# linusmossberg/monte-carlo-ray-tracer

Measured on NVIDIA H100. Metric: Mray/s (primary+shadow+bounce), higher is better.
Workload: dtype f64

## Files before the change

monte-carlo-ray-tracer_b200/csrc/abi.cu:

```cuda
#include <algorithm>
#include <cmath>
#include <cstdio>
#include <cstdlib>
#include <cstring>
#include <string>
#include <vector>

#include "mcrt_abi.h"
#include "launch.h"
#include "bvh_build.h"
#include "image.h"
#include "denoise.h"

using namespace mcrt;

static const int MCRT_INTERNAL_EMIT = 100;

#define CK(call)                                                                              \
    do {                                                                                      \
        cudaError_t e_ = (call);                                                              \
        if (e_ != cudaSuccess)                                                                \
        {                                                                                     \
            ctx->error = std::string(#call) + ": " + cudaGetErrorString(e_);                  \
            return MCRT_ERR_CUDA;                                                             \
// ... 489 lines not shown
        for (uint32_t i = 0; i < s.n_prims; i++)
        {
            if (s.prim_type[i] == MCRT_PRIM_SPHERE && d.prims_class == PRIMS_TRI) d.prims_class = PRIMS_TRI_SPHERE;
            else if (s.prim_type[i] != MCRT_PRIM_TRIANGLE && s.prim_type[i] != MCRT_PRIM_SPHERE) { d.prims_class = PRIMS_ALL; break; }
        }
        d.material_flags_any = 0;
        for (const auto& m : a.materials) d.material_flags_any |= m.flags;
        d.scene_ior = (R)s.scene_ior;
        d.scene_scale = (R)ctx->scene_scale;
        return MCRT_OK;
    }

    template <class R>
    int ensureWave(mcrt_ctx* ctx, WaveBuffers<R>& w, std::vector<void*>& track)
    {
        if (w.capacity == ctx->pool_paths) return MCRT_OK;
        freeAll(track);
        w.capacity = 0;
        const size_t n = ctx->pool_paths;
        int rc;
        for (int b = 0; b < 2; b++)
        {
            if ((rc = devAlloc(ctx, track, &w.buf[b].ray_o, n))) return rc;
            if ((rc = devAlloc(ctx, track, &w.buf[b].ray_d, n))) return rc;
            if ((rc = devAlloc(ctx, track, &w.buf[b].thr, n))) return rc;
            if ((rc = devAlloc(ctx, track, &w.buf[b].iors_a, n))) return rc;
            if ((rc = devAlloc(ctx, track, &w.buf[b].iors_b, n))) return rc;
            if ((rc = devAlloc(ctx, track, &w.buf[b].meta, n))) return rc;
            if ((rc = devAlloc(ctx, track, &w.buf[b].meta2, n))) return rc;
        }
        if ((rc = devAlloc(ctx, track, &w.shadow, n))) return rc;
        if ((rc = devAlloc(ctx, track, &w.hits, n))) return rc;
        w.capacity = ctx->pool_paths;
        return MCRT_OK;
    }

    int ensureSort(mcrt_ctx* ctx)
    {
        if (ctx->sort_capacity == ctx->pool_paths) return MCRT_OK;
        freeAll(ctx->sort_allocs);
        ctx->sort_capacity = 0;
        const size_t n = ctx->pool_paths;
        int rc;
        RaySort& r = ctx->sort;
        for (int b = 0; b < 2; b++)
        {
            if ((rc = devAlloc(ctx, ctx->sort_allocs, &r.path_key[b], n))) return rc;
            if ((rc = devAlloc(ctx, ctx->sort_allocs, &r.path_rank[b], n))) return rc;
        }
        if ((rc = devAlloc(ctx, ctx->sort_allocs, &r.path_order, n))) return rc;
        if ((rc = devAlloc(ctx, ctx->sort_allocs, &r.shadow_key, n))) return rc;
        if ((rc = devAlloc(ctx, ctx->sort_allocs, &r.shadow_rank, n))) return rc;
        if ((rc = devAlloc(ctx, ctx->sort_allocs, &r.shadow_order, n))) return rc;
        if ((rc = devAlloc(ctx, ctx->sort_allocs, &r.shade_key, n))) return rc;
        if ((rc = devAlloc(ctx, ctx->sort_allocs, &r.shade_rank, n))) return rc;
        if ((rc = devAlloc(ctx, ctx->sort_allocs, &r.shade_order, n))) return rc;
        if ((rc = devAlloc(ctx, ctx->sort_allocs, &r.hist_shade, (size_t)SORT_BINS))) return rc;
        if ((rc = devAlloc(ctx, ctx->sort_allocs, &r.hist_path, (size_t)SORT_BINS))) return rc;
        if ((rc = devAlloc(ctx, ctx->sort_allocs, &r.hist_shadow, (size_t)SORT_BINS))) return rc;
        if ((rc = devAlloc(ctx, ctx->sort_allocs, &r.bin_start, (size_t)SORT_BINS))) return rc;
        if ((rc = devAlloc(ctx, ctx->sort_allocs, &r.block_offset, (size_t)2 * SORT_SCAN_BLOCKS))) return rc;
        if ((rc = devAlloc(ctx, ctx->sort_allocs, &r.done_counter, (size_t)1))) return rc;
        CK(cudaMemset(r.done_counter, 0, sizeof(uint32_t)));
        ctx->sort_capacity = ctx->pool_paths;
        return MCRT_OK;
    }

    int ensureFilm(mcrt_ctx* ctx, size_t values)
    {
        if (ctx->film_values >= values && ctx->d_film) return MCRT_OK;
        if (ctx->d_film) cudaFree(ctx->d_film);
        ctx->d_film = nullptr; ctx->film_values = 0;
        CK(cudaMalloc((void**)&ctx->d_film, values * sizeof(double)));
        ctx->film_values = values;
        return MCRT_OK;
    }

    template <class R> DeviceScene<R>& sceneOf(mcrt_ctx* ctx);
    template <> DeviceScene<double>& sceneOf<double>(mcrt_ctx* ctx) { return ctx->scene64; }
    template <> DeviceScene<float>& sceneOf<float>(mcrt_ctx* ctx) { return ctx->scene32; }
    template <class R> WaveBuffers<R>& waveOf(mcrt_ctx* ctx);
    template <> WaveBuffers<double>& waveOf<double>(mcrt_ctx* ctx) { return ctx->wave64; }
    template <> WaveBuffers<float>& waveOf<float>(mcrt_ctx* ctx) { return ctx->wave32; }
    template <class R> std::vector<void*>& waveAllocsOf(mcrt_ctx* ctx);
    template <> std::vector<void*>& waveAllocsOf<double>(mcrt_ctx* ctx) { return ctx->wave_allocs64; }
    template <> std::vector<void*>& waveAllocsOf<float>(mcrt_ctx* ctx) { return ctx->wave_allocs32; }

    void fillStats(mcrt_stats* st, const Counters& c, uint64_t iterations, uint64_t launches, double ms)
    {
        if (!st) return;
        std::memset(st, 0, sizeof(*st));
        st->paths = c.paths;
        st->extension_rays = c.extension_rays;
        st->shadow_rays = c.shadow_rays;
        st->box_tests = c.box_tests;
        st->prim_tests = c.prim_tests;
        st->knn_queries = c.knn_queries;
        st->wavefront_iterations = iterations;
        st->kernel_launches = launches;
        st->ior_stack_overflows = c.ior_stack_overflows;
        st->max_depth = c.max_depth;
        st->gpu_ms_total = ms;
        st->shadow_box_tests = c.shadow_box_tests;
        st->shadow_prim_tests = c.shadow_prim_tests;
        st->extend_work_sum = c.work_sum;
        st->extend_work_warpmax = c.work_warpmax;
        st->replayed_rays = c.replayed_rays;
    }
// ... 162 lines not shown
        CK(cudaEventRecord(ctx->ev_start, s));
        CK(cudaMemcpyAsync(ctx->d_counters, &ctx->h_counters[0], sizeof(Counters), cudaMemcpyHostToDevice, s));
        if (!accum)
        {
            CK(cudaMemsetAsync(ctx->d_film, 0, film_pixels * 3 * sizeof(double), s));
            if (filtered) CK(cudaMemsetAsync(ctx->d_film_wsum, 0, film_pixels * sizeof(double), s));
        }
        const bool sorting = ctx->sort_rays != 0;
        if (sorting)
        {
            CK(cudaMemsetAsync(p.sort.hist_path, 0, SORT_BINS * sizeof(uint32_t), s));
            CK(cudaMemsetAsync(p.sort.hist_shadow, 0, SORT_BINS * sizeof(uint32_t), s));
            CK(cudaMemsetAsync(ctx->sort.hist_shade, 0, SORT_BINS * sizeof(uint32_t), s));
        }
        auto sortPaths = [&](int buffer)
        {
            launchSortScan(p.sort.hist_path, p.sort, s);
            launchSortScatter(p.sort.path_key[buffer], p.sort.path_rank[buffer], p.sort, p.sort.path_order,
                              &ctx->d_counters->n_cur, grid, s);
        };

        uint64_t launches = 0, iterations = 0;

        if (emitting) Launch<R>::emitGenerate(p, 0, grid, s);
        else Launch<R>::generate(p, 0, grid, s);
        launchAdvance(ctx->d_counters, s);
        launches += 2;
        if (sorting) { sortPaths(0); launches += 2; }

        int pending[2] = { 0, 0 };
        int slot = 0;
        bool done = false;
        while (!done)
        {
            for (int k = 0; k < ctx->poll_interval; k++)
            {
                const int cur = (int)(iterations & 1u);
                cudaEvent_t* ev = nullptr;
                if (ctx->stage_timing)
                {
                    while (ctx->stage_events.size() < 6 * (iterations + 1))
                    {
                        cudaEvent_t e;
                        CK(cudaEventCreate(&e));
                        ctx->stage_events.push_back(e);
                    }
                    ev = &ctx->stage_events[6 * iterations];
                    cudaEventRecord(ev[0], s);
                }
                Launch<R>::extend(p, cur, grid, s);
                if (ev) cudaEventRecord(ev[1], s);
                if (p.sort.shade_order)
                {
                    Launch<R>::shadeKey(p, grid, s);
                    launchSortScan(p.sort.hist_shade, p.sort, s);
                    launchSortScatter(p.sort.shade_key, p.sort.shade_rank, p.sort, p.sort.shade_order, &ctx->d_counters->n_cur, grid, s);
                    launches += 3;
                }
                if (emitting)
                {
                    Launch<R>::emitShade(p, cur, grid, s);
                }
                else if (integrator == MCRT_INTEGRATOR_PHOTON)
                {
                    Launch<R>::shadePhoton(p, cur, grid, s);
                    if (ev) cudaEventRecord(ev[5], s);
                    Launch<R>::knn(p, grid, s);
                    launches += 1;
                }
                else
                {
                    Launch<R>::shade(p, cur, grid, s);
                }
                if (ev) cudaEventRecord(ev[2], s);
                if (!emitting)
                {
                    if (sorting)
                    {
                        launchSortScan(p.sort.hist_shadow, p.sort, s);
                        launchSortScatter(p.sort.shadow_key, p.sort.shadow_rank, p.sort, p.sort.shadow_order,
                                          &ctx->d_counters->n_shadow, grid, s);
                        launches += 2;
                    }
                    Launch<R>::shadow(p, grid, s);
                }
                if (ev) cudaEventRecord(ev[3], s);
                if (emitting) Launch<R>::emitGenerate(p, cur ^ 1, grid, s);
                else Launch<R>::generate(p, cur ^ 1, grid, s);
                launchAdvance(ctx->d_counters, s);
                if (sorting) { sortPaths(cur ^ 1); launches += 2; }
                if (ev) cudaEventRecord(ev[4], s);
                launches += 5;
                iterations++;
            }
            CK(cudaMemcpyAsync(&ctx->h_counters[slot], ctx->d_counters, sizeof(Counters), cudaMemcpyDeviceToHost, s));
            CK(cudaEventRecord(ctx->ev_poll[slot], s));
            pending[slot] = 1;
            const int other = slot ^ 1;
            if (pending[other])
            {
                CK(cudaEventSynchronize(ctx->ev_poll[other]));
                const Counters& c = ctx->h_counters[other];
                if (c.n_cur == 0 && c.next_work >= c.total_work) done = true;
                pending[other] = 0;
            }
            slot = other;
        }

        if (!emitting && !accum)
        {
// ... 1514 lines not shown
```

monte-carlo-ray-tracer_b200/csrc/integrator.cuh:

```cuda
#pragma once

#include "bsdf.cuh"
#include "intersect.cuh"
#include "bvh4.cuh"
#include "photon.cuh"
#include "film.cuh"
#include "mcrt_abi.h"

#ifndef MCRT_TRACE_MINBLOCKS_F64
#define MCRT_TRACE_MINBLOCKS_F64 2
#endif
#ifndef MCRT_TRACE_MINBLOCKS_F32
#define MCRT_TRACE_MINBLOCKS_F32 4
#endif
#ifndef MCRT_TRACE_MINBLOCKS_F64_PRUNED
#define MCRT_TRACE_MINBLOCKS_F64_PRUNED 4
#endif
#ifndef MCRT_TRACE_MINBLOCKS_FAST
#define MCRT_TRACE_MINBLOCKS_FAST 2
#endif
#ifndef MCRT_TRACE_MINBLOCKS_DYN
#define MCRT_TRACE_MINBLOCKS_DYN 4
#endif
#ifndef MCRT_KNN_MINBLOCKS
#define MCRT_KNN_MINBLOCKS 8
#endif
#ifndef MCRT_GATHER_MINBLOCKS
#define MCRT_GATHER_MINBLOCKS 3
#endif
#ifndef MCRT_SHADE_MINBLOCKS
#define MCRT_SHADE_MINBLOCKS 3
#endif
#ifndef MCRT_SHADE_MINBLOCKS_LITE
#define MCRT_SHADE_MINBLOCKS_LITE 3
#endif
#ifndef MCRT_SORT_ORIGIN_BITS
#define MCRT_SORT_ORIGIN_BITS 4
#endif
#ifndef MCRT_SORT_DIR_Q
#define MCRT_SORT_DIR_Q 1
#endif

namespace mcrt
{
    constexpr int IOR_STACK_CAPACITY = 8;

    struct Counters
    {
        uint32_t n_cur, n_next, n_shadow, n_gen;
        unsigned long long next_work, total_work;
        unsigned long long paths, extension_rays, shadow_rays, box_tests, prim_tests, knn_queries;
        unsigned long long shadow_box_tests, shadow_prim_tests;
        unsigned long long ior_stack_overflows;
        unsigned long long replayed_rays;
        uint32_t fetch_extend, fetch_shadow;
        uint32_t traversal_overflow, max_depth;
        uint32_t n_knn, _pad;
        unsigned long long work_sum, work_warpmax;
        unsigned long long n_photons[2];
        uint32_t photon_overflow, _pad2;
    };

    template <class R> struct PathBuffer
    {
        V4<R>* ray_o;
        V4<R>* ray_d;
        V4<R>* thr;
        V4<R>* iors_a;
        V4<R>* iors_b;
        uint4* meta;
        uint4* meta2;
    };

    template <class R> struct alignas(16 * sizeof(R)) ShadowRecord
    {
        V4<R> o;
        V4<R> d;
        uint4 meta;
        V4<R> k;
    };
    static_assert(sizeof(ShadowRecord<double>) == 128 && sizeof(ShadowRecord<float>) == 64, "one shadow record per line");
    static_assert(offsetof(ShadowRecord<double>, k) == 96, "the float64 padding is the 16-byte chunk 5 (k_shade writes it)");

    constexpr uint32_t SORT_ORIGIN_BITS = MCRT_SORT_ORIGIN_BITS;
    constexpr uint32_t SORT_DIR_Q = MCRT_SORT_DIR_Q;
    constexpr uint32_t SORT_DIR_BITS = 3 + 2 * SORT_DIR_Q;
    constexpr uint32_t SORT_KEY_BITS = 3 * SORT_ORIGIN_BITS + SORT_DIR_BITS;
    constexpr uint32_t SORT_BINS = 1u << SORT_KEY_BITS;

    struct RaySort
    {
        uint32_t* path_key[2];
        uint32_t* path_rank[2];
        uint32_t* path_order;
        uint32_t* shadow_key;
        uint32_t* shadow_rank;
        uint32_t* shadow_order;
        uint32_t* hist_path;
        uint32_t* hist_shadow;
        uint32_t* bin_start;
        uint32_t* block_offset;
        uint32_t* done_counter;
        uint32_t shade_sorted;
        uint32_t* shade_key;
        uint32_t* shade_rank;
        uint32_t* shade_order;
        uint32_t* hist_shade;
        uint32_t prim_scale;
        float key_min[3], key_scale[3];
    };

    MCRT_D uint32_t spreadBits3(uint32_t v)
    {
        v = (v | (v << 16)) & 0x030000FFu;
        v = (v | (v << 8)) & 0x0300F00Fu;
        v = (v | (v << 4)) & 0x030C30C3u;
        v = (v | (v << 2)) & 0x09249249u;
        return v;
    }

    template <class R>
    MCRT_D uint32_t rayKey(const RaySort& rs, const V3<R>& o, const V3<R>& d, uint32_t src_prim)
    {
        uint32_t cell;
        if (rs.prim_scale && src_prim != NO_PRIM)
        {
            cell = (uint32_t)(((unsigned long long)src_prim * rs.prim_scale) >> 32);
        }
        else
        {
            constexpr float CELLS = (float)(1u << SORT_ORIGIN_BITS);
            float cx = ((float)o.x - rs.key_min[0]) * rs.key_scale[0];
            float cy = ((float)o.y - rs.key_min[1]) * rs.key_scale[1];
            float cz = ((float)o.z - rs.key_min[2]) * rs.key_scale[2];
            uint32_t ix = (uint32_t)fminf(fmaxf(cx, 0.0f), CELLS - 1.0f);
            uint32_t iy = (uint32_t)fminf(fmaxf(cy, 0.0f), CELLS - 1.0f);
            uint32_t iz = (uint32_t)fminf(fmaxf(cz, 0.0f), CELLS - 1.0f);
            cell = spreadBits3(ix) | (spreadBits3(iy) << 1) | (spreadBits3(iz) << 2);
        }
        float dx = (float)d.x, dy = (float)d.y, dz = (float)d.z;
        float ax = fabsf(dx), ay = fabsf(dy), az = fabsf(dz);
        uint32_t face; float u, v, m;
        if (ax >= ay && ax >= az) { face = dx < 0.0f ? 1u : 0u; u = dy; v = dz; m = ax; }
        else if (ay >= az)        { face = dy < 0.0f ? 3u : 2u; u = dx; v = dz; m = ay; }
        else                      { face = dz < 0.0f ? 5u : 4u; u = dx; v = dy; m = az; }
        constexpr float Q = (float)(1u << SORT_DIR_Q);
        float inv = m > 0.0f ? 0.5f * Q / m : 0.0f;
        uint32_t qu = (uint32_t)fminf(fmaxf(u * inv + 0.5f * Q, 0.0f), Q - 1.0f);
        uint32_t qv = (uint32_t)fminf(fmaxf(v * inv + 0.5f * Q, 0.0f), Q - 1.0f);
        uint32_t dir = (face << (2 * SORT_DIR_Q)) | (qu << SORT_DIR_Q) | qv;
        return (dir << (3 * SORT_ORIGIN_BITS)) | cell;
    }

    MCRT_D uint32_t sortRank(uint32_t* hist, uint32_t key, bool pred)
    {
        const unsigned active = __ballot_sync(0xFFFFFFFFu, pred);
        uint32_t rank = 0;
        if (pred)
// ... 255 lines not shown
            {
            const unsigned long long w = base_work + j;
            uint32_t pixel, sample, film_index;
            V3<R> start, direction;
            if (p.user_rays)
            {
                pixel = p.user_pixel[w];
                sample = p.user_sample[w];
                film_index = (uint32_t)w;
                const double* r = p.user_rays + 6 * w;
                start = V3<R>((R)r[0], (R)r[1], (R)r[2]);
                direction = V3<R>((R)r[3], (R)r[4], (R)r[5]);
            }
            else
            {
                uint32_t local = (uint32_t)(w % p.n_pixels);
                if constexpr (LIST) local = p.pixel_list[local];
                sample = (uint32_t)(w / p.n_pixels);
                const uint32_t row = local / p.camera.width, col = local - row * p.camera.width;
                pixel = (p.row_first + row * p.row_step) * p.camera.width + col;
                film_index = local;
                SamplerState smp = SamplerState::make(p.global_seed, pixel, sample, 0u);
                cameraRay(p.camera, p.scene.scene_ior, pixel, smp, start, direction);
                if constexpr (FILM) filmSplatSampleWeight(p.filmp, p.global_seed, pixel, sample);
            }
            stStream(&out.ray_o[slot], V4<R>(start, p.scene.scene_ior));
            stStream(&out.ray_d[slot], V4<R>(direction, R(1)));
            stStream(&out.thr[slot], V4<R>(R(1), R(1), R(1), R(0)));
            stStream(&out.meta[slot], make_uint4(pixel, sample, 0u, 0u));
            stStream(&out.meta2[slot], make_uint4(NO_PRIM, 1u, film_index, NO_PRIM));
            if (p.sort.path_order) key = rayKey(p.sort, start, direction, NO_PRIM);
            }
            if (p.sort.path_order)
            {
                const uint32_t rank = sortRank(p.sort.hist_path, key, valid);
                if (valid) { p.sort.path_key[next][slot] = key; p.sort.path_rank[next][slot] = rank; }
            }
        }
    }

    static __global__ void k_advance(Counters* c)
    {
        c->n_cur = c->n_next + c->n_gen;
        c->next_work += c->n_gen;
        c->paths += c->n_gen;
        c->n_next = 0;
        c->n_gen = 0;
        c->n_shadow = 0;
        c->n_knn = 0;
        c->fetch_extend = 0;
        c->fetch_shadow = 0;
    }

    template <class R, int PRIMS, int FAST>
    __global__ void __launch_bounds__(256, FAST == 2 ? MCRT_TRACE_MINBLOCKS_DYN : (FAST == 1 ? MCRT_TRACE_MINBLOCKS_FAST : (PRIMS == PRIMS_ALL ? Mode<R>::trace_minblocks : Mode<R>::trace_minblocks_pruned))) k_extend(WaveParams<R> p, int cur)
    {
        const uint32_t n = p.counters->n_cur;
        const PathBuffer<R>& in = p.buf[cur];
        TraceCounters cnt = { 0u, 0u, 0u };
        uint32_t overflow = 0;
        unsigned long long rays = 0;
        const uint32_t* order = p.sort.path_order;
        if constexpr (Mode<R>::parity && FAST == 2)
        {
            traceManyFast<PRIMS>(p.scene, n, &p.counters->fetch_extend,
                [&](uint32_t ii, RayQ<R>& r)
                {
                    const uint32_t i = order ? order[ii] : ii;
                    const V4<R> ro = ldStream(&in.ray_o[i]), rd = ldStream(&in.ray_d[i]);
                    r.o = ro.xyz(); r.d = rd.xyz();
                    if constexpr (PRIMS == PRIMS_ALL) r.inv_d = R(1) / r.d;
                    return i;
                },
                [&](uint32_t i, const RayQ<R>&, const Hit<R>& h)
                {
                    stStream(&p.hits[i], V4<R>(h.t, h.u, h.v, h.prim == NO_PRIM ? R(-1) : R(h.prim)));
                    rays++;
                }, cnt, overflow);
            flushStats(p.counters, cnt, rays, false, overflow);
            return;
        }
        for (uint32_t ii = blockIdx.x * blockDim.x + threadIdx.x; ii < n; ii += gridDim.x * blockDim.x)
        {
            const uint32_t i = order ? order[ii] : ii;
            const V4<R> ro = ldStream(&in.ray_o[i]);
            const V4<R> rd = ldStream(&in.ray_d[i]);
            uint32_t skip = NO_PRIM;
            if constexpr (!Mode<R>::parity) skip = in.meta2[i].w;
#ifdef MCRT_TAIL_DIAGNOSTIC
            const uint32_t w0 = cnt.box_tests + cnt.prim_tests;
#endif
            Hit<R> h = traceClosest<PRIMS, FAST != 0>(p.scene, ro.xyz(), rd.xyz(), skip, cnt, overflow);
            stStream(&p.hits[i], V4<R>(h.t, h.u, h.v, h.prim == NO_PRIM ? R(-1) : R(h.prim)));
            rays++;
#ifdef MCRT_TAIL_DIAGNOSTIC
            const uint32_t w = cnt.box_tests + cnt.prim_tests - w0;
            const unsigned am = __activemask();
            const uint32_t wmax = __reduce_max_sync(am, w);
            atomicAdd(&p.counters->work_sum, (unsigned long long)w);
            if ((threadIdx.x & 31u) == (unsigned)(__ffs(am) - 1)) atomicAdd(&p.counters->work_warpmax, 32ull * wmax);
#endif
        }
        flushStats(p.counters, cnt, rays, false, overflow);
    }

    template <class R>
    MCRT_D void sampleLightPoint(const Light<R>& l, R u, R v, V3<R>& pos, V3<R>& normal)
    {
        if (l.type == PRIM_TRIANGLE)
        {
            R su = msqrt(u);
            pos = (R(1) - su) * l.p0 + (R(1) - v) * su * l.p1 + v * su * l.p2;
            normal = l.normal;
        }
        else
        {
            R z = R(1) - R(2) * u;
            R r = msqrt(R(1) - pow2(z));
            R phi = Consts<R>::TWO_PI * v;
            R sn, cs;
            msincos(phi, &sn, &cs);
            pos = l.p0 + l.p1.x * V3<R>(r * cs, r * sn, z);
            normal = (pos - l.p0) / l.p1.x;
        }
    }

    template <class R> MCRT_D R powerHeuristic(R a_pdf, R b_pdf)
    {
        R a2 = a_pdf * a_pdf;
        return a2 / (a2 + b_pdf * b_pdf);
    }

    template <class R> MCRT_D V3<R> skyColor(const V3<R>& dir)
    {
        R d = R(0) * dir.x + R(1) * dir.y + R(0) * dir.z;
        if constexpr (sizeof(R) == 4) d = gclamp(d, R(-1), R(1));
        R fy = (R(1) + masin(d) / Consts<R>::PI) / R(2);
        return mix(V3<R>(R(1), R(0.5), R(0)), V3<R>(R(0), R(0.5), R(1)), fy);
    }

    constexpr uint32_t SHADE_FEATS_ALL = 0xFFFFFFFFu;
    constexpr uint32_t SHADE_FEATS_LITE = ~(uint32_t)(MAT_ROUGH | MAT_ROUGH_SPECULAR | MAT_COMPLEX_IOR);

    template <class R, int KIND, int FILM, uint32_t FEATS>
    __global__ void __launch_bounds__(128, FEATS == 0xFFFFFFFFu ? MCRT_SHADE_MINBLOCKS : MCRT_SHADE_MINBLOCKS_LITE) k_shade(WaveParams<R> p, int cur)
    {
        __shared__ SobolByteTables sobol_tab;
        sobol_tab.fill(p.sobol_bytes);
        __syncthreads();
        Counters* c = p.counters;
        const uint32_t n = c->n_cur;
        const PathBuffer<R>& in = p.buf[cur];
        const PathBuffer<R>& out = p.buf[cur ^ 1];
        const DeviceScene<R>& sc = p.scene;
        uint32_t local_max_depth = 0;
        uint32_t stack_overflows = 0;
// ... 182 lines not shown
                                    sh_area_cos = L.area * cos_light_theta;
                                    sh_select = ls_select;
                                    sh_light = L.prim;
                                    if constexpr (FILM == FILM_MODE_AOV) sh_plane = aovPlane(lobe, ray.depth > 0u, false);
                                }
                            }
                        }
                    }

                    V3<R> bsdf_absIdotN;
                    if (!do_bsdf)
                    {
                    }
                    else if (!sampleBSDF(ia, ray, smp, p.ray_eps, false, bsdf_absIdotN, ls_bsdf_pdf, nray))
                    {
                        alive = false;
                    }
                    else
                    {
                        throughput *= bsdf_absIdotN / ls_bsdf_pdf;
                        R survive = compMax(throughput) * nray.refraction_scale;
                        if (survive == R(0))
                        {
                            alive = false;
                        }
                        else if (nray.diffuse_depth > 3u || nray.depth > 16u)
                        {
                            survive = gmin(R(0.95), survive);
                            R ua;
                            samplerGet<R, DIM_ABSORB, 1>(smp, &ua);
                            if (survive <= ua) alive = false;
                            else throughput /= survive;
                        }
                    }

                    if (alive)
                    {
                        if (nray.refraction_level > 0)
                        {
                            if (nray.refraction_level == (int32_t)ior_count)
                            {
                                if (ior_count < (uint32_t)IOR_STACK_CAPACITY) iors[ior_count++] = nray.medium_ior;
                                else stack_overflows++;
                            }
                            else if (nray.refraction_level < (int32_t)ior_count - 1)
                            {
                                ior_count--;
                            }
                        }
                    }
                }
            }

            const uint32_t slot = warpAppend(&c->n_next, alive);
            const uint32_t sslot = warpAppend(&c->n_shadow, want_shadow);
            uint32_t pkey = 0, prank = 0, skey = 0, srank = 0;
            if (sorting && alive)
            {
                pkey = rayKey(p.sort, nray.start, nray.direction, hit_prim);
                prank = atomicAdd(&p.sort.hist_path[pkey], 1u);
            }
            if (sorting && want_shadow)
            {
                skey = rayKey(p.sort, sh_o, sh_d, hit_prim);
                srank = atomicAdd(&p.sort.hist_shadow[skey], 1u);
            }
            if (alive)
            {
                stStream(&out.ray_o[slot], V4<R>(nray.start, nray.medium_ior));
                stStream(&out.ray_d[slot], V4<R>(nray.direction, nray.refraction_scale));
                stStream(&out.thr[slot], V4<R>(throughput, ls_bsdf_pdf));
                if (ior_count > 1)
                {
                    out.iors_a[slot] = V4<R>(iors[1], iors[2], iors[3], iors[4]);
                    if (ior_count > 5) out.iors_b[slot] = V4<R>(iors[5], iors[6], iors[7], R(0));
                }
                stStream(&out.meta[slot], make_uint4(meta.x, meta.y, (nray.depth & 0xFFFFu) | (nray.diffuse_depth << 16),
                                                     (uint32_t)nray.refraction_level));
                stStream(&out.meta2[slot], make_uint4(ls_light, ior_count | (nray.dirac_delta ? 256u : 0u) | (lobe << 9), meta2.z,
                                                      sc.shade[hit_prim].type == PRIM_TRIANGLE ? hit_prim : NO_PRIM));
                if (sorting) { p.sort.path_key[cur ^ 1][slot] = pkey; p.sort.path_rank[cur ^ 1][slot] = prank; }
            }
            if (want_shadow)
            {
                ShadowRecord<R>& srec = p.shadow[sslot];
                stStream(&srec.o, V4<R>(sh_o, sh_bsdf_pdf));
                stStream(&srec.d, V4<R>(sh_d, sh_area_cos));
                stStream(&srec.meta, make_uint4(sh_light, meta2.z, sc.shade[hit_prim].type == PRIM_TRIANGLE ? hit_prim : NO_PRIM,
                                                FILM == FILM_MODE_AOV ? sh_plane : meta.y));
                if constexpr (sizeof(R) == 8) stStream(reinterpret_cast<uint4*>(&srec) + 5, make_uint4(0u, 0u, 0u, 0u));
                stStream(&srec.k, V4<R>(sh_k, sh_select));
                if (sorting) { p.sort.shadow_key[sslot] = skey; p.sort.shadow_rank[sslot] = srank; }
            }

            if constexpr (KIND == 1)
            {
                const uint32_t q0 = warpAppend(&c->n_knn, want_knn >= 1);
                if (want_knn >= 1 && q0 < p.pm.query_capacity) p.pm.queries[q0] = knn_q;
                const uint32_t q1 = warpAppend(&c->n_knn, want_knn == 2);
                if (want_knn == 2 && q1 < p.pm.query_capacity)
                {
                    knn_q.meta.z |= 2u;
                    p.pm.queries[q1] = knn_q;
                }
            }
        }

        if (local_max_depth) atomicMax(&c->max_depth, local_max_depth);
        if (stack_overflows) atomicAdd(&c->ior_stack_overflows, (unsigned long long)stack_overflows);
    }

    template <class R, int FILM, int PRIMS, int FAST>
    __global__ void __launch_bounds__(256, FAST == 2 ? MCRT_TRACE_MINBLOCKS_DYN : (FAST == 1 ? MCRT_TRACE_MINBLOCKS_FAST : (PRIMS == PRIMS_ALL ? Mode<R>::trace_minblocks : Mode<R>::trace_minblocks_pruned))) k_shadow(WaveParams<R> p)
    {
        const uint32_t n = p.counters->n_shadow;
        TraceCounters cnt = { 0u, 0u, 0u };
        uint32_t overflow = 0;
        unsigned long long rays = 0;
// ... 1 lines not shown
        if constexpr (Mode<R>::parity && FAST == 2)
        {
            traceManyFast<PRIMS, true>(p.scene, n, &p.counters->fetch_shadow,
                [&](uint32_t ii, RayQ<R>& r, uint32_t& target)
                {
                    const uint32_t i = order ? order[ii] : ii;
                    const V4<R> so = ldStream(&p.shadow[i].o), sd = ldStream(&p.shadow[i].d);
                    r.o = so.xyz(); r.d = sd.xyz();
                    if constexpr (PRIMS == PRIMS_ALL) r.inv_d = R(1) / r.d;
                    target = p.shadow[i].meta.x;
                    return i;
                },
                [&](uint32_t i, const RayQ<R>&, const Hit<R>& h)
                {
                    rays++;
                    const ShadowRecord<R>& srec = p.shadow[i];
                    const uint4 sm = srec.meta;
                    if (h.prim == sm.x)
                    {
                        const V4<R> so = srec.o, sd = srec.d, sk = srec.k;
                        R light_pdf = pow2(h.t) / sd.w;
                        R mis_weight = powerHeuristic(light_pdf, so.w);
                        depositRadiance<FILM>(p, sm.y, pixelOfFilmIndex(p, sm.y), sm.w, sk.xyz() * (mis_weight / (light_pdf * sk.w)),
                                              FILM == FILM_MODE_GROUPS ? p.scene.shade[sm.x].light : NO_PRIM, sm.w);
                    }
                }, cnt, overflow);
            flushStats(p.counters, cnt, rays, true, overflow);
            return;
        }
        for (uint32_t ii = blockIdx.x * blockDim.x + threadIdx.x; ii < n; ii += gridDim.x * blockDim.x)
        {
            const uint32_t i = order ? order[ii] : ii;
            const ShadowRecord<R>& srec = p.shadow[i];
            const V4<R> so = ldStream(&srec.o), sd = ldStream(&srec.d);
            const uint4 sm = ldStream(&srec.meta);
            Hit<R> h;
            if constexpr (Mode<R>::parity && FAST != 0) h = traceVisible<PRIMS>(p.scene, so.xyz(), sd.xyz(), sm.x, cnt, overflow);
            else h = traceClosest<PRIMS, false>(p.scene, so.xyz(), sd.xyz(), sm.z, cnt, overflow);
            rays++;
            if (h.prim == sm.x)
            {
                const V4<R> sk = srec.k;
                R light_pdf = pow2(h.t) / sd.w;
                R mis_weight = powerHeuristic(light_pdf, so.w);
                depositRadiance<FILM>(p, sm.y, pixelOfFilmIndex(p, sm.y), sm.w, sk.xyz() * (mis_weight / (light_pdf * sk.w)),
                                      FILM == FILM_MODE_GROUPS ? p.scene.shade[sm.x].light : NO_PRIM, sm.w);
            }
        }
        flushStats(p.counters, cnt, rays, true, overflow);
    }



    constexpr uint32_t SHADE_CLASS_BINS = 64;

    template <class R>
    __global__ void __launch_bounds__(256) k_shade_key(WaveParams<R> p)
    {
        __shared__ uint32_t s_hist[SHADE_CLASS_BINS], s_base[SHADE_CLASS_BINS];
        const uint32_t n = p.counters->n_cur;
        const uint32_t chunks = (n + 255u) / 256u;
        for (uint32_t chunk = blockIdx.x; chunk < chunks; chunk += gridDim.x)
        {
            if (threadIdx.x < SHADE_CLASS_BINS) s_hist[threadIdx.x] = 0u;
            __syncthreads();
            const uint32_t i = chunk * 256u + threadIdx.x;
            uint32_t key = 0, local = 0;
            if (i < n)
            {
                const R w = p.hits[i].w;
                if (!(w < R(0))) key = p.scene.shade_class[(uint32_t)w];
                local = atomicAdd(&s_hist[key], 1u);
            }
            __syncthreads();
            if (threadIdx.x < SHADE_CLASS_BINS && s_hist[threadIdx.x]) s_base[threadIdx.x] = atomicAdd(&p.sort.hist_shade[threadIdx.x], s_hist[threadIdx.x]);
            __syncthreads();
            if (i < n) { p.sort.shade_key[i] = key; p.sort.shade_rank[i] = s_base[key] + local; }
            __syncthreads();
        }
    }

    constexpr uint32_t SORT_SCAN_BLOCKS = SORT_BINS / 1024;

    static __global__ void __launch_bounds__(256) k_sort_scan(uint32_t* hist, uint32_t* bin_start, uint32_t* block_offset,
                                                              uint32_t* done_counter)
    {
        __shared__ uint32_t warp_sums[8];
        __shared__ uint32_t is_last;
        const uint32_t t = threadIdx.x, base = blockIdx.x * 1024u + t * 4u;
        const uint4 v = *reinterpret_cast<const uint4*>(hist + base);
        *reinterpret_cast<uint4*>(hist + base) = make_uint4(0u, 0u, 0u, 0u);
        const uint32_t sum = v.x + v.y + v.z + v.w;
        uint32_t incl = sum;
        for (int off = 1; off < 32; off <<= 1)
        {
            const uint32_t u = __shfl_up_sync(0xFFFFFFFFu, incl, off);
            if ((t & 31u) >= (uint32_t)off) incl += u;
        }
        if ((t & 31u) == 31u) warp_sums[t >> 5] = incl;
        __syncthreads();
        uint32_t warp_base = 0;
        for (uint32_t w = 0; w < (t >> 5); w++) warp_base += warp_sums[w];
        const uint32_t excl = warp_base + incl - sum;
        *reinterpret_cast<uint4*>(bin_start + base) = make_uint4(excl, excl + v.x, excl + v.x + v.y, excl + v.x + v.y + v.z);
        if (t == 255u)
        {
            block_offset[SORT_SCAN_BLOCKS + blockIdx.x] = excl + sum;
            __threadfence();
            is_last = atomicAdd(done_counter, 1u) == gridDim.x - 1u;
        }
        __syncthreads();
        if (is_last && t < 32u)
        {
            __threadfence();
            constexpr uint32_t PER_LANE = SORT_SCAN_BLOCKS / 32;
            uint32_t lane_sum = 0;
            for (uint32_t k = 0; k < PER_LANE; k++) lane_sum += block_offset[SORT_SCAN_BLOCKS + t * PER_LANE + k];
            uint32_t inc = lane_sum;
            for (int off = 1; off < 32; off <<= 1)
            {
                const uint32_t u = __shfl_up_sync(0xFFFFFFFFu, inc, off);
                if (t >= (uint32_t)off) inc += u;
            }
            uint32_t run = inc - lane_sum;
            for (uint32_t k = 0; k < PER_LANE; k++)
            {
                const uint32_t tot = block_offset[SORT_SCAN_BLOCKS + t * PER_LANE + k];
                block_offset[t * PER_LANE + k] = run;
                run += tot;
            }
            if (t == 0) *done_counter = 0u;
// ... 607 lines not shown
```

monte-carlo-ray-tracer_b200/csrc/kernels_impl.cuh:

```cuda
#include "launch.h"

namespace mcrt
{
    template <> void Launch<MCRT_REAL>::generate(const WaveParams<MCRT_REAL>& p, int next, int grid, cudaStream_t s)
    {
        if (p.pixel_list)
        {
            if (p.filmp.is_default_box) k_generate<MCRT_REAL, false, true><<<grid, 256, 0, s>>>(p, next);
            else k_generate<MCRT_REAL, true, true><<<grid, 256, 0, s>>>(p, next);
            return;
        }
        if (p.filmp.is_default_box) k_generate<MCRT_REAL, false, false><<<grid, 256, 0, s>>>(p, next);
        else k_generate<MCRT_REAL, true, false><<<grid, 256, 0, s>>>(p, next);
    }
    template <> void Launch<MCRT_REAL>::extend(const WaveParams<MCRT_REAL>& p, int cur, int grid, cudaStream_t s)
    {
        if constexpr (Mode<MCRT_REAL>::parity)
        {
            if (p.scene.bvh4 && p.scene.dynamic_fetch)
            {
                if (p.scene.prims_class == PRIMS_TRI) k_extend<MCRT_REAL, PRIMS_TRI, 2><<<grid, 256, fastStackSharedBytes(256), s>>>(p, cur);
                else if (p.scene.prims_class == PRIMS_TRI_SPHERE) k_extend<MCRT_REAL, PRIMS_TRI_SPHERE, 2><<<grid, 256, fastStackSharedBytes(256), s>>>(p, cur);
                else k_extend<MCRT_REAL, PRIMS_ALL, 2><<<grid, 256, fastStackSharedBytes(256), s>>>(p, cur);
                return;
// ... 59 lines not shown
            do { static bool attr_set = false; \
                 if (!attr_set) { cudaFuncSetAttribute(k_knn<MCRT_REAL, SL, false, FE>, cudaFuncAttributeMaxDynamicSharedMemorySize, (int)knnSharedBytes(1024)); attr_set = true; } \
                 k_knn<MCRT_REAL, SL, false, FE><<<g, b, smem, s>>>(p); } while (0)
        #define MCRT_KNN_LAUNCH(SL) \
            do { if (lite) MCRT_KNN_LAUNCH1(SL, SHADE_FEATS_LITE); else MCRT_KNN_LAUNCH1(SL, SHADE_FEATS_ALL); } while (0)
        switch (slots)
        {
            case 1: MCRT_KNN_LAUNCH(1); break;
            case 2: MCRT_KNN_LAUNCH(2); break;
            case 4: MCRT_KNN_LAUNCH(4); break;
            case 8: MCRT_KNN_LAUNCH(8); break;
            default: MCRT_KNN_LAUNCH(0); break;
        }
        #undef MCRT_KNN_LAUNCH
        #undef MCRT_KNN_LAUNCH1
    }
    template <int FILM> static void launchShadowBox(const WaveParams<MCRT_REAL>& p, int grid, cudaStream_t s)
    {
        if constexpr (Mode<MCRT_REAL>::parity)
        {
            if (p.scene.bvh4 && p.scene.dynamic_fetch)
            {
                if (p.scene.prims_class == PRIMS_TRI) k_shadow<MCRT_REAL, FILM, PRIMS_TRI, 2><<<grid, 256, fastStackSharedBytes(256), s>>>(p);
                else if (p.scene.prims_class == PRIMS_TRI_SPHERE) k_shadow<MCRT_REAL, FILM, PRIMS_TRI_SPHERE, 2><<<grid, 256, fastStackSharedBytes(256), s>>>(p);
                else k_shadow<MCRT_REAL, FILM, PRIMS_ALL, 2><<<grid, 256, fastStackSharedBytes(256), s>>>(p);
                return;
            }
            if (p.scene.bvh4)
            {
                if (p.scene.prims_class == PRIMS_TRI) k_shadow<MCRT_REAL, FILM, PRIMS_TRI, 1><<<grid, 256, fastStackSharedBytes(256), s>>>(p);
                else if (p.scene.prims_class == PRIMS_TRI_SPHERE) k_shadow<MCRT_REAL, FILM, PRIMS_TRI_SPHERE, 1><<<grid, 256, fastStackSharedBytes(256), s>>>(p);
                else k_shadow<MCRT_REAL, FILM, PRIMS_ALL, 1><<<grid, 256, fastStackSharedBytes(256), s>>>(p);
                return;
            }
        }
        if (p.scene.prims_class == PRIMS_TRI) k_shadow<MCRT_REAL, FILM, PRIMS_TRI, 0><<<grid, 256, 0, s>>>(p);
        else if (p.scene.prims_class == PRIMS_TRI_SPHERE) k_shadow<MCRT_REAL, FILM, PRIMS_TRI_SPHERE, 0><<<grid, 256, 0, s>>>(p);
        else k_shadow<MCRT_REAL, FILM, PRIMS_ALL, 0><<<grid, 256, 0, s>>>(p);
    }
    template <> void Launch<MCRT_REAL>::shadow(const WaveParams<MCRT_REAL>& p, int grid, cudaStream_t s)
    {
        if (!p.filmp.is_default_box)
        {
            if constexpr (Mode<MCRT_REAL>::parity)
            {
                if (p.scene.bvh4) { k_shadow<MCRT_REAL, FILM_MODE_SPLAT, PRIMS_ALL, 1><<<grid, 256, fastStackSharedBytes(256), s>>>(p); return; }
            }
            k_shadow<MCRT_REAL, FILM_MODE_SPLAT, PRIMS_ALL, 0><<<grid, 256, 0, s>>>(p);
        }
        else if (p.n_planes && p.aovs) launchShadowBox<FILM_MODE_AOV>(p, grid, s);
        else if (p.n_planes) launchShadowBox<FILM_MODE_GROUPS>(p, grid, s);
        else launchShadowBox<FILM_MODE_BOX>(p, grid, s);
    }
    template <> void Launch<MCRT_REAL>::shadeKey(const WaveParams<MCRT_REAL>& p, int grid, cudaStream_t s)
    {
        k_shade_key<MCRT_REAL><<<grid, 256, 0, s>>>(p);
    }
    template <> void Launch<MCRT_REAL>::emitGenerate(const WaveParams<MCRT_REAL>& p, int next, int grid, cudaStream_t s)
    {
        k_emit_generate<MCRT_REAL><<<grid, 256, 0, s>>>(p, next);
    }
    template <> void Launch<MCRT_REAL>::emitShade(const WaveParams<MCRT_REAL>& p, int cur, int grid, cudaStream_t s)
    {
        k_emit_shade<MCRT_REAL><<<grid * 2, 128, 0, s>>>(p, cur);
    }
    template <> void Launch<MCRT_REAL>::traceUser(const DeviceScene<MCRT_REAL>& sc, const double* rays6, size_t n,
                                                  double* out_tuv, uint32_t* out_prim, Counters* c, int grid, cudaStream_t s)
    {
        if constexpr (Mode<MCRT_REAL>::parity)
        {
            if (sc.bvh4) { k_trace_user<MCRT_REAL, true><<<grid, 256, fastStackSharedBytes(256), s>>>(sc, rays6, n, out_tuv, out_prim, c); return; }
        }
        k_trace_user<MCRT_REAL, false><<<grid, 256, 0, s>>>(sc, rays6, n, out_tuv, out_prim, c);
    }
    template <> void Launch<MCRT_REAL>::features(const DeviceScene<MCRT_REAL>& sc, const DeviceCamera<MCRT_REAL>& cam, uint32_t global_seed,
                                                 uint32_t sample_first, uint32_t sample_count, double* out, Counters* c, int grid,
                                                 cudaStream_t s)
    {
        if constexpr (Mode<MCRT_REAL>::parity)
        {
            if (sc.bvh4) { k_features<MCRT_REAL, true><<<grid, 256, fastStackSharedBytes(256), s>>>(sc, cam, global_seed, sample_first, sample_count, out, c); return; }
        }
        k_features<MCRT_REAL, false><<<grid, 256, 0, s>>>(sc, cam, global_seed, sample_first, sample_count, out, c);
    }
    template <> void Launch<MCRT_REAL>::featuresChain(const DeviceScene<MCRT_REAL>& sc, const DeviceCamera<MCRT_REAL>& cam, uint32_t global_seed,
                                                      uint32_t sample_first, uint32_t sample_count, uint32_t specular_depth,
                                                      MCRT_REAL ray_eps, double* out, Counters* c, int grid, cudaStream_t s)
    {
        if constexpr (Mode<MCRT_REAL>::parity)
        {
            if (sc.bvh4)
            {
                k_features_chain<MCRT_REAL, true><<<grid, 256, fastStackSharedBytes(256), s>>>(sc, cam, global_seed, sample_first, sample_count,
                                                                                              specular_depth, ray_eps, out, c);
                return;
            }
        }
        k_features_chain<MCRT_REAL, false><<<grid, 256, 0, s>>>(sc, cam, global_seed, sample_first, sample_count, specular_depth, ray_eps, out, c);
    }
}
```

monte-carlo-ray-tracer_b200/csrc/launch.h:

```cpp
#pragma once

#include "integrator.cuh"

namespace mcrt
{
    template <class R> struct Launch
    {
        static void generate(const WaveParams<R>& p, int next, int grid, cudaStream_t s);
        static void extend(const WaveParams<R>& p, int cur, int grid, cudaStream_t s);
        static void shade(const WaveParams<R>& p, int cur, int grid, cudaStream_t s);
        static void shadePhoton(const WaveParams<R>& p, int cur, int grid, cudaStream_t s);
        static void knn(const WaveParams<R>& p, int grid, cudaStream_t s);
        static void emitGenerate(const WaveParams<R>& p, int next, int grid, cudaStream_t s);
        static void emitShade(const WaveParams<R>& p, int cur, int grid, cudaStream_t s);
        static void shadow(const WaveParams<R>& p, int grid, cudaStream_t s);
        static void shadeKey(const WaveParams<R>& p, int grid, cudaStream_t s);
        static void traceUser(const DeviceScene<R>& sc, const double* rays6, size_t n, double* out_tuv,
                              uint32_t* out_prim, Counters* c, int grid, cudaStream_t s);
        static void features(const DeviceScene<R>& sc, const DeviceCamera<R>& cam, uint32_t global_seed, uint32_t sample_first,
                             uint32_t sample_count, double* out, Counters* c, int grid, cudaStream_t s);
        static void featuresChain(const DeviceScene<R>& sc, const DeviceCamera<R>& cam, uint32_t global_seed, uint32_t sample_first,
                                  uint32_t sample_count, uint32_t specular_depth, R ray_eps, double* out, Counters* c, int grid,
                                  cudaStream_t s);
    };

    void launchAdvance(Counters* c, cudaStream_t s);
    void launchSortScan(uint32_t* hist, const RaySort& rs, cudaStream_t s);
    void launchSortScatter(const uint32_t* key, const uint32_t* rank, const RaySort& rs, uint32_t* order,
                           const uint32_t* n_ptr, int grid, cudaStream_t s);
    void launchResolveFilmWeighted(const double* film, const double* wsum, double* out, size_t n_pixels, int grid, cudaStream_t s);
    void launchResolveFilm(const double* film, double* out, size_t n_values, double weight, int grid, cudaStream_t s);
    void launchResolveFilmPeers(const double* film, const PeerFrames& pf, size_t n_values, double weight, int grid, cudaStream_t s);
    void launchProgressiveResolve(const ProgressiveHalf& a, const ProgressiveHalf& b, bool weighted, uint32_t width, uint32_t rows,
                                  uint32_t tile, uint32_t tiles_x, double* out, double* sums, double* tile_error, uint32_t n_tiles,
                                  int grid, cudaStream_t s, const double* tile_counts = nullptr);
    void launchLightGroupsCombine(const double* planes, uint32_t n_planes, uint64_t n_values, const double* weights, double* out,
                                  int grid, cudaStream_t s);
    void launchFp64Peak(double* sink, int iterations, int grid, cudaStream_t s);
    void launchKnnUser(const DevicePhotonMap& map, uint32_t k, const double* points, size_t n, uint32_t* out_index,
                       double* out_d2, uint32_t* out_count, uint32_t* overflow_flag, int grid, cudaStream_t s);
    void launchGatherUser(const DevicePhotonMap& map, const double* points, size_t n, double r2, uint32_t* out_count,
                          double* out_flux, double* out_cone, uint32_t* overflow_flag, int grid, cudaStream_t s);
    void launchSamplerStream(const uint32_t* pixel, const uint32_t* sample, size_t n, uint32_t n_shuffles,
                             uint32_t global_seed, uint32_t* out, cudaStream_t s);
}
```

Before: 2717.

## Fuse shade-class histogram into extend and replace three-pass shade sort with one kernel

The extend kernel now builds a per-block shared-memory histogram of shade classes and flushes it to the global histogram, so the separate key kernel, scan kernel and scatter kernel for shading order collapse into a single kernel. That kernel scans the 64-bin histogram in one warp and scatters path indices directly, using a done-counter to reset the histogram. Separately, the shade kernel's queue appends and sort-rank atomics are warp-aggregated with ballot and match_any so one leader lane per key does each atomic. This trades extra shared atomics in extend and a last-block handshake for fewer launches and less global traffic.

```diff
diff --git a/monte-carlo-ray-tracer_b200/csrc/abi.cu b/monte-carlo-ray-tracer_b200/csrc/abi.cu
--- a/monte-carlo-ray-tracer_b200/csrc/abi.cu
+++ b/monte-carlo-ray-tracer_b200/csrc/abi.cu
@@ -565,8 +565,6 @@
         if ((rc = devAlloc(ctx, ctx->sort_allocs, &r.shadow_key, n))) return rc;
         if ((rc = devAlloc(ctx, ctx->sort_allocs, &r.shadow_rank, n))) return rc;
         if ((rc = devAlloc(ctx, ctx->sort_allocs, &r.shadow_order, n))) return rc;
-        if ((rc = devAlloc(ctx, ctx->sort_allocs, &r.shade_key, n))) return rc;
-        if ((rc = devAlloc(ctx, ctx->sort_allocs, &r.shade_rank, n))) return rc;
         if ((rc = devAlloc(ctx, ctx->sort_allocs, &r.shade_order, n))) return rc;
         if ((rc = devAlloc(ctx, ctx->sort_allocs, &r.hist_shade, (size_t)SORT_BINS))) return rc;
         if ((rc = devAlloc(ctx, ctx->sort_allocs, &r.hist_path, (size_t)SORT_BINS))) return rc;
@@ -835,10 +833,8 @@
                 if (ev) cudaEventRecord(ev[1], s);
                 if (p.sort.shade_order)
                 {
-                    Launch<R>::shadeKey(p, grid, s);
-                    launchSortScan(p.sort.hist_shade, p.sort, s);
-                    launchSortScatter(p.sort.shade_key, p.sort.shade_rank, p.sort, p.sort.shade_order, &ctx->d_counters->n_cur, grid, s);
-                    launches += 3;
+                    Launch<R>::shadeClassOrder(p, grid, s);
+                    launches += 1;
                 }
                 if (emitting)
                 {
diff --git a/monte-carlo-ray-tracer_b200/csrc/integrator.cuh b/monte-carlo-ray-tracer_b200/csrc/integrator.cuh
--- a/monte-carlo-ray-tracer_b200/csrc/integrator.cuh
+++ b/monte-carlo-ray-tracer_b200/csrc/integrator.cuh
@@ -34,6 +34,9 @@
 #ifndef MCRT_SHADE_MINBLOCKS_LITE
 #define MCRT_SHADE_MINBLOCKS_LITE 3
 #endif
+#ifndef MCRT_SHADE_AGGREGATE_RANKS
+#define MCRT_SHADE_AGGREGATE_RANKS 1
+#endif
 #ifndef MCRT_SORT_ORIGIN_BITS
 #define MCRT_SORT_ORIGIN_BITS 4
 #endif
@@ -102,8 +105,6 @@
         uint32_t* block_offset;
         uint32_t* done_counter;
         uint32_t shade_sorted;
-        uint32_t* shade_key;
-        uint32_t* shade_rank;
         uint32_t* shade_order;
         uint32_t* hist_shade;
         uint32_t prim_scale;
@@ -465,6 +466,14 @@
         c->fetch_shadow = 0;
     }
 
+    constexpr uint32_t SHADE_CLASS_BINS = 64;
+
+    template <class R>
+    MCRT_D uint32_t shadeClassOf(const DeviceScene<R>& sc, uint32_t prim)
+    {
+        return prim == NO_PRIM ? 0u : sc.shade_class[prim];
+    }
+
     template <class R, int PRIMS, int FAST>
     __global__ void __launch_bounds__(256, FAST == 2 ? MCRT_TRACE_MINBLOCKS_DYN : (FAST == 1 ? MCRT_TRACE_MINBLOCKS_FAST : (PRIMS == PRIMS_ALL ? Mode<R>::trace_minblocks : Mode<R>::trace_minblocks_pruned))) k_extend(WaveParams<R> p, int cur)
     {
@@ -474,6 +483,20 @@
         uint32_t overflow = 0;
         unsigned long long rays = 0;
         const uint32_t* order = p.sort.path_order;
+        __shared__ uint32_t s_class[SHADE_CLASS_BINS];
+        const bool classes = p.sort.shade_order != nullptr;
+        if (classes)
+        {
+            for (uint32_t k = threadIdx.x; k < SHADE_CLASS_BINS; k += blockDim.x) s_class[k] = 0u;
+            __syncthreads();
+        }
+        auto flushClasses = [&]()
+        {
+            if (!classes) return;
+            __syncthreads();
+            for (uint32_t k = threadIdx.x; k < SHADE_CLASS_BINS; k += blockDim.x)
+                if (s_class[k]) atomicAdd(&p.sort.hist_shade[k], s_class[k]);
+        };
         if constexpr (Mode<R>::parity && FAST == 2)
         {
             traceManyFast<PRIMS>(p.scene, n, &p.counters->fetch_extend,
@@ -488,9 +511,11 @@
                 [&](uint32_t i, const RayQ<R>&, const Hit<R>& h)
                 {
                     stStream(&p.hits[i], V4<R>(h.t, h.u, h.v, h.prim == NO_PRIM ? R(-1) : R(h.prim)));
+                    if (classes) atomicAdd(&s_class[shadeClassOf(p.scene, h.prim)], 1u);
                     rays++;
                 }, cnt, overflow);
             flushStats(p.counters, cnt, rays, false, overflow);
+            flushClasses();
             return;
         }
         for (uint32_t ii = blockIdx.x * blockDim.x + threadIdx.x; ii < n; ii += gridDim.x * blockDim.x)
@@ -505,6 +530,7 @@
 #endif
             Hit<R> h = traceClosest<PRIMS, FAST != 0>(p.scene, ro.xyz(), rd.xyz(), skip, cnt, overflow);
             stStream(&p.hits[i], V4<R>(h.t, h.u, h.v, h.prim == NO_PRIM ? R(-1) : R(h.prim)));
+            if (classes) atomicAdd(&s_class[shadeClassOf(p.scene, h.prim)], 1u);
             rays++;
 #ifdef MCRT_TAIL_DIAGNOSTIC
             const uint32_t w = cnt.box_tests + cnt.prim_tests - w0;
@@ -515,6 +541,7 @@
 #endif
         }
         flushStats(p.counters, cnt, rays, false, overflow);
+        flushClasses();
     }
 
     template <class R>
@@ -803,18 +830,42 @@
                 }
             }
 
-            const uint32_t slot = warpAppend(&c->n_next, alive);
-            const uint32_t sslot = warpAppend(&c->n_shadow, want_shadow);
+            const unsigned lane = threadIdx.x & 31u, lower = (1u << lane) - 1u;
+            const unsigned amask = __ballot_sync(0xFFFFFFFFu, alive), smask = __ballot_sync(0xFFFFFFFFu, want_shadow);
             uint32_t pkey = 0, prank = 0, skey = 0, srank = 0;
-            if (sorting && alive)
-            {
-                pkey = rayKey(p.sort, nray.start, nray.direction, hit_prim);
-                prank = atomicAdd(&p.sort.hist_path[pkey], 1u);
-            }
-            if (sorting && want_shadow)
-            {
-                skey = rayKey(p.sort, sh_o, sh_d, hit_prim);
-                srank = atomicAdd(&p.sort.hist_shadow[skey], 1u);
+            unsigned ppeers = 0, speers = 0;
+            if (sorting)
+            {
+                if (alive) pkey = rayKey(p.sort, nray.start, nray.direction, hit_prim);
+                if (want_shadow) skey = rayKey(p.sort, sh_o, sh_d, hit_prim);
+#if MCRT_SHADE_AGGREGATE_RANKS
+                ppeers = __match_any_sync(0xFFFFFFFFu, alive ? pkey : 0xFFFFFFFFu);
+                speers = __match_any_sync(0xFFFFFFFFu, want_shadow ? skey : 0xFFFFFFFFu);
+#else
+                ppeers = 1u << lane; speers = 1u << lane;
+#endif
+#ifdef MCRT_SHADE_KEY_STATS
+                const unsigned pm = __match_any_sync(0xFFFFFFFFu, alive ? pkey : 0xFFFFFFFFu);
+                const unsigned sm = __match_any_sync(0xFFFFFFFFu, want_shadow ? skey : 0xFFFFFFFFu);
+                const uint32_t dp = __popc(__ballot_sync(0xFFFFFFFFu, alive && (pm & lower) == 0u));
+                const uint32_t ds = __popc(__ballot_sync(0xFFFFFFFFu, want_shadow && (sm & lower) == 0u));
+                if (lane == 0u && dp) atomicAdd(&c->work_sum, (1ull << 36) + dp);
+                if (lane == 0u && ds) atomicAdd(&c->work_warpmax, (1ull << 36) + ds);
+#endif
+            }
+            uint32_t qbase = 0, sbase = 0;
+            if (amask && lane == (unsigned)(__ffs(amask) - 1)) qbase = atomicAdd(&c->n_next, (uint32_t)__popc(amask));
+            if (smask && lane == (unsigned)(__ffs(smask) - 1)) sbase = atomicAdd(&c->n_shadow, (uint32_t)__popc(smask));
+            const int pleader = __ffs(ppeers) - 1, sleader = __ffs(speers) - 1;
+            if (sorting && alive && (int)lane == pleader) prank = atomicAdd(&p.sort.hist_path[pkey], (uint32_t)__popc(ppeers));
+            if (sorting && want_shadow && (int)lane == sleader) srank = atomicAdd(&p.sort.hist_shadow[skey], (uint32_t)__popc(speers));
+            if (amask) qbase = __shfl_sync(0xFFFFFFFFu, qbase, __ffs(amask) - 1);
+            if (smask) sbase = __shfl_sync(0xFFFFFFFFu, sbase, __ffs(smask) - 1);
+            const uint32_t slot = qbase + __popc(amask & lower), sslot = sbase + __popc(smask & lower);
+            if (sorting)
+            {
+                prank = __shfl_sync(0xFFFFFFFFu, prank, pleader < 0 ? (int)lane : pleader) + __popc(ppeers & lower);
+                srank = __shfl_sync(0xFFFFFFFFu, srank, sleader < 0 ? (int)lane : sleader) + __popc(speers & lower);
             }
             if (alive)
             {
@@ -922,31 +973,55 @@
 
 
 
-    constexpr uint32_t SHADE_CLASS_BINS = 64;
-
     template <class R>
-    __global__ void __launch_bounds__(256) k_shade_key(WaveParams<R> p)
-    {
-        __shared__ uint32_t s_hist[SHADE_CLASS_BINS], s_base[SHADE_CLASS_BINS];
+    __global__ void __launch_bounds__(256) k_shade_class_order(WaveParams<R> p)
+    {
+        __shared__ uint32_t s_start[SHADE_CLASS_BINS], s_hist[SHADE_CLASS_BINS], s_base[SHADE_CLASS_BINS];
+        __shared__ uint32_t is_last;
+        uint32_t* hist = p.sort.hist_shade;
+        const uint32_t t = threadIdx.x;
         const uint32_t n = p.counters->n_cur;
+        if (t < 32u)
+        {
+            const uint32_t a = hist[2u * t], b = hist[2u * t + 1u];
+            uint32_t incl = a + b;
+            for (int off = 1; off < 32; off <<= 1)
+            {
+                const uint32_t u = __shfl_up_sync(0xFFFFFFFFu, incl, off);
+                if (t >= (uint32_t)off) incl += u;
+            }
+            s_start[2u * t] = incl - a - b;
+            s_start[2u * t + 1u] = incl - b;
+        }
         const uint32_t chunks = (n + 255u) / 256u;
         for (uint32_t chunk = blockIdx.x; chunk < chunks; chunk += gridDim.x)
         {
-            if (threadIdx.x < SHADE_CLASS_BINS) s_hist[threadIdx.x] = 0u;
+            if (t < SHADE_CLASS_BINS) s_hist[t] = 0u;
             __syncthreads();
-            const uint32_t i = chunk * 256u + threadIdx.x;
-            uint32_t key = 0, local = 0;
+            const uint32_t i = chunk * 256u + t;
+            uint32_t k = 0, local = 0;
             if (i < n)
             {
                 const R w = p.hits[i].w;
-                if (!(w < R(0))) key = p.scene.shade_class[(uint32_t)w];
-                local = atomicAdd(&s_hist[key], 1u);
+                k = shadeClassOf(p.scene, w < R(0) ? NO_PRIM : (uint32_t)w);
+                local = atomicAdd(&s_hist[k], 1u);
             }
             __syncthreads();
-            if (threadIdx.x < SHADE_CLASS_BINS && s_hist[threadIdx.x]) s_base[threadIdx.x] = atomicAdd(&p.sort.hist_shade[threadIdx.x], s_hist[threadIdx.x]);
+            if (t < SHADE_CLASS_BINS && s_hist[t]) s_base[t] = s_start[t] + atomicAdd(&hist[SHADE_CLASS_BINS + t], s_hist[t]);
             __syncthreads();
-            if (i < n) { p.sort.shade_key[i] = key; p.sort.shade_rank[i] = s_base[key] + local; }
+            if (i < n) p.sort.shade_order[s_base[k] + local] = i;
             __syncthreads();
+        }
+        if (t == 0)
+        {
+            __threadfence();
+            is_last = atomicAdd(p.sort.done_counter, 1u) == gridDim.x - 1u;
+        }
+        __syncthreads();
+        if (is_last)
+        {
+            if (t < 2u * SHADE_CLASS_BINS) hist[t] = 0u;
+            if (t == 0) *p.sort.done_counter = 0u;
         }
     }
 
diff --git a/monte-carlo-ray-tracer_b200/csrc/kernels_impl.cuh b/monte-carlo-ray-tracer_b200/csrc/kernels_impl.cuh
--- a/monte-carlo-ray-tracer_b200/csrc/kernels_impl.cuh
+++ b/monte-carlo-ray-tracer_b200/csrc/kernels_impl.cuh
@@ -135,9 +135,9 @@
         else if (p.n_planes) launchShadowBox<FILM_MODE_GROUPS>(p, grid, s);
         else launchShadowBox<FILM_MODE_BOX>(p, grid, s);
     }
-    template <> void Launch<MCRT_REAL>::shadeKey(const WaveParams<MCRT_REAL>& p, int grid, cudaStream_t s)
+    template <> void Launch<MCRT_REAL>::shadeClassOrder(const WaveParams<MCRT_REAL>& p, int grid, cudaStream_t s)
     {
-        k_shade_key<MCRT_REAL><<<grid, 256, 0, s>>>(p);
+        k_shade_class_order<MCRT_REAL><<<grid, 256, 0, s>>>(p);
     }
     template <> void Launch<MCRT_REAL>::emitGenerate(const WaveParams<MCRT_REAL>& p, int next, int grid, cudaStream_t s)
     {
diff --git a/monte-carlo-ray-tracer_b200/csrc/launch.h b/monte-carlo-ray-tracer_b200/csrc/launch.h
--- a/monte-carlo-ray-tracer_b200/csrc/launch.h
+++ b/monte-carlo-ray-tracer_b200/csrc/launch.h
@@ -14,7 +14,7 @@
         static void emitGenerate(const WaveParams<R>& p, int next, int grid, cudaStream_t s);
         static void emitShade(const WaveParams<R>& p, int cur, int grid, cudaStream_t s);
         static void shadow(const WaveParams<R>& p, int grid, cudaStream_t s);
-        static void shadeKey(const WaveParams<R>& p, int grid, cudaStream_t s);
+        static void shadeClassOrder(const WaveParams<R>& p, int grid, cudaStream_t s);
         static void traceUser(const DeviceScene<R>& sc, const double* rays6, size_t n, double* out_tuv,
                               uint32_t* out_prim, Counters* c, int grid, cudaStream_t s);
         static void features(const DeviceScene<R>& sc, const DeviceCamera<R>& cam, uint32_t global_seed, uint32_t sample_first,
```

Result: faster. 2762, median of 6 (+1.7%).
